# alibaba/nann

Hardware: AMD Instinct MI355X
Metric: retrieval QPS @ recall@200 parity, 1M items/128-d (higher is better)
Workload: dtype f16 rows / f32 L2

## Files before the change

nann_amd/build.py:

```python
import os
import subprocess
import sys

HERE = os.path.dirname(os.path.abspath(__file__))
SRC_DIR = os.path.join(HERE, "csrc")
OUT_DIR = os.path.join(HERE, "_build")
LIB = os.path.join(OUT_DIR, "libnann_hip.so")
UNITS = [("nann_core.o", [("nann_hip.hip", {}), ("nann_comm.hip", {}), ("nann_hnsw_build.hip", {})]),
         ("nann_l2_f16.o", [("nann_l2_inst.hip", {"NANN_L2_DT": "0", "NANN_L2_NAME": "f16"})]),
         ("nann_l2_bf16.o", [("nann_l2_inst.hip", {"NANN_L2_DT": "1", "NANN_L2_NAME": "bf16"})]),
         ("nann_l2_f32.o", [("nann_l2_inst.hip", {"NANN_L2_DT": "2", "NANN_L2_NAME": "f32"})]),
         ("nann_mlp_d64_res.o", [("nann_mlp_inst.hip", {"NANN_MLP_D": "64"}), ("nann_mlp_res_inst.hip", {})]),
         ("nann_mlp_d128.o", [("nann_mlp_inst.hip", {"NANN_MLP_D": "128"})]),
         ("nann_mlp_d256.o", [("nann_mlp_inst.hip", {"NANN_MLP_D": "256"})]),
         ("nann_attn.o", [("nann_attn_inst.hip", {})]),
         ("nann_attn_split.o", [("nann_attn_split_inst.hip", {})]),
         ("nann_eval.o", [("nann_eval_inst.hip", {})]),
         ("nann_eval_lds.o", [("nann_eval_lds_inst.hip", {})]),
         ("nann_eval_win.o", [("nann_eval_win_inst.hip", {})])]
DEPS = ["nann_hip.hip", "nann_mlp_inst.hip", "nann_mlp_res_inst.hip", "nann_mlp5.h", "nann_mlp6.h", "nann_l2_inst.hip", "nann_attn_inst.hip", "nann_attn_split_inst.hip", "nann_attn_split.h", "nann_attn_proj.h", "nann_eval_inst.hip", "nann_eval_lds_inst.hip", "nann_eval_win_inst.hip", "nann_eval.h", "nann_comm.hip", "nann_hnsw_build.hip", "nann_device.h", "nann_mlp.h", "nann_mlp2.h", "nann_mlp3.h",
        "nann_attn.h", "nann_attn_kernels.h", "nann_search.h", os.path.join("host", "nann_graphdef.h"), os.path.join("host", "nann_graphdef_text.h"), os.path.join("host", "nann_blaze_options.h"), os.path.join("host", "nann_npy.h"), os.path.join("host", "nann_projcache.h"),
        os.path.join("..", "..", "include", "nann_hip.h")]
FLAGS = ["-O3", "-std=c++17", "--offload-arch=gfx950", "-fPIC", "-fno-fast-math", "-ffp-contract=off"]


def _hipcc():
    for c in (os.environ.get("HIPCC"), "/opt/rocm/bin/hipcc", "hipcc"):
        if c and (os.path.isabs(c) and os.path.exists(c) or not os.path.isabs(c)):
            return c
    return "hipcc"


def source_hash():
    import hashlib
    h = hashlib.sha256()
    for d in sorted(DEPS):
        with open(os.path.join(SRC_DIR, d), "rb") as f:
            h.update(d.encode() + b"\0" + f.read())
    h.update(" ".join(FLAGS).encode())
    return h.hexdigest()


def is_stale():
    if not os.path.exists(LIB):
        return True
    try:
        with open(LIB + ".srchash") as f:
            return f.read().strip() != source_hash()
    except OSError:
        return True


def build(force=False, verbose=False, variant=None, extra_flags=()):
    if variant is None:
# ... 86 lines not shown
```

nann_amd/csrc/nann_hip.hip:

```cpp
#include "nann_eval.h"
#include "nann_attn.h"
#include "host/nann_graphdef_text.h"
#include "host/nann_blaze_options.h"
#include "host/nann_npy.h"
#include "host/nann_projcache.h"

#include <algorithm>
#include <atomic>
#include <cmath>
#include <cstdio>
#include <cstdlib>
#include <cstring>
#include <fstream>
#include <memory>
#include <mutex>
#include <string>
#include <vector>

#include <sys/stat.h>

using namespace nann;

namespace nann {
thread_local std::string g_err;
int fail(int code, const std::string& msg) {
  g_err = msg;
  return code;
}
}

namespace {

#define HIP_TRY(expr)                                                                    \
  do {                                                                                   \
// ... 578 lines not shown
struct HipProjBackend {
  typedef hipStream_t Stream;
  typedef hipEvent_t Event;
  static bool malloc(void** p, size_t bytes) {
    if (hipMalloc(p, bytes) == hipSuccess) return true;
    (void)hipGetLastError();
    return false;
  }
  static void free(void* p) { (void)hipFree(p); }
  static bool mem_info(size_t* free_b) {
    size_t total = 0;
    if (hipMemGetInfo(free_b, &total) == hipSuccess) return true;
    (void)hipGetLastError();
    return false;
  }
  static bool event_create(Event* e) {
    if (hipEventCreateWithFlags(e, hipEventDisableTiming) == hipSuccess) return true;
    (void)hipGetLastError();
    return false;
  }
  static void event_destroy(Event e) { (void)hipEventDestroy(e); }
  static void event_record(Event e, Stream s) { (void)hipEventRecord(e, s); }
  static bool event_done(Event e) { return hipEventQuery(e) != hipErrorNotReady; }
  static void event_wait(Event e) { (void)hipEventSynchronize(e); }
};
typedef nann::ProjCacheT<HipProjBackend> ProjCache;
typedef nann::ProjTableT<HipProjBackend> ProjTable;
struct SearchOpt {
  int mode;
  int reserve;
  int preproject;
  int mlp_form;
  int small32;
};
static std::atomic<int> g_traversal_mode{-1}, g_slot_reserve{-1}, g_preproject{-1};
static const SearchOpt& env_defaults() {
  static const SearchOpt d = [] {
    SearchOpt o{NANN_TRAVERSAL_AUTO, 0, 1, NANN_MLP_FORM_AUTO, 1};
    if (const char* e = std::getenv("NANN_PREPROJECT")) o.preproject = !(e[0] == '0' && e[1] == 0);
    if (const char* e = std::getenv("NANN_SEARCH_SLOT_RESERVE")) o.reserve = std::max(0, std::atoi(e));
    if (const char* e = std::getenv("NANN_MLP_FORM")) o.mlp_form = std::string(e) == "fused" ? NANN_MLP_FORM_FUSED : std::string(e) == "phased" ? NANN_MLP_FORM_PHASED : NANN_MLP_FORM_AUTO;
    if (const char* e = std::getenv("NANN_PHASE_SMALL32")) o.small32 = !(e[0] == '0');
    return o;
  }();
  return d;
}
static SearchOpt resolve_options(const nann_search_options* u) {
  SearchOpt o = env_defaults();
  const int gm = g_traversal_mode.load(std::memory_order_relaxed), gr = g_slot_reserve.load(std::memory_order_relaxed),
            gp = g_preproject.load(std::memory_order_relaxed);
  if (gm >= 0) o.mode = gm;
  if (gr >= 0) o.reserve = gr;
  if (gp >= 0) o.preproject = gp;
  if (u) {
    const size_t nb = u->struct_bytes > 0 ? (size_t)u->struct_bytes : sizeof(*u);
    auto has = [&](const int32_t* f) { return (size_t)(reinterpret_cast<const char*>(f) - reinterpret_cast<const char*>(u)) + 4 <= nb; };
    if (has(&u->traversal_mode) && u->traversal_mode >= 0) o.mode = u->traversal_mode;
    if (has(&u->slot_reserve) && u->slot_reserve >= 0) o.reserve = u->slot_reserve;
    if (has(&u->preprojection) && u->preprojection >= 0) o.preproject = u->preprojection != 0;
    if (has(&u->mlp_form) && u->mlp_form >= 0) o.mlp_form = u->mlp_form;
  }
  return o;
}
static int check_options(const nann_search_options* u) {
  if (!u) return NANN_OK;
  if (u->struct_bytes < 0 || (u->struct_bytes > 0 && u->struct_bytes < 8)) return fail(NANN_ERR_BAD_ARGUMENT, "nann_search_options: struct_bytes");
  const SearchOpt o = resolve_options(u);
  if (o.mode < NANN_TRAVERSAL_AUTO || o.mode > NANN_TRAVERSAL_LDS_HASH32) return fail(NANN_ERR_BAD_ARGUMENT, "nann_search_options: unknown traversal_mode");
  if (o.mlp_form < NANN_MLP_FORM_AUTO || o.mlp_form > NANN_MLP_FORM_PHASED) return fail(NANN_ERR_BAD_ARGUMENT, "nann_search_options: unknown mlp_form");
  return NANN_OK;
}

struct nann_scorer {
  nann_scorer_desc desc;
  float* dev_weights = nullptr;
  uint4* dev_packed = nullptr;
  float4* dev_packed_x = nullptr;
  MlpParams mlp = {};
  mutable ProjCache proj;
};

struct nann_attn_scorer {
  AttnParams P = {};
  int emb_dtype = 0;
  int precision = NANN_MLP_EXACT_F32;
  float* dev_weights = nullptr;
  uint4* dev_packed = nullptr;
  mutable ProjCache proj;
};

struct nann_index {
  nann_index_desc desc;
  uint64_t uid = 0;
  bool owns = false;
  std::vector<void*> owned;
  int64_t max_deg[2] = {0, 0};
  uint32_t bm_words = 0;
  bool probe_valid = false;
  int probe_ef = 0, probe_queries = 0;
  float probe_new_per_row_mean = 0.0f, probe_new_per_row_q90 = 0.0f, probe_new_per_row_max = 0.0f;
};
static void probe_index(nann_index* ix);

extern "C" {

int nann_abi_version(void) { return NANN_ABI_VERSION; }
const char* nann_last_error(void) { return nann::g_err.c_str(); }

int nann_device_count(void) {
  int n = 0;
  if (hipGetDeviceCount(&n) != hipSuccess) return 0;
  return n;
}

int nann_malloc(void** dev_ptr, int64_t nbytes) {
  if (!dev_ptr || nbytes < 0) return fail(NANN_ERR_BAD_ARGUMENT, "nann_malloc: bad argument");
  HIP_TRY(hipMalloc(dev_ptr, (size_t)std::max<int64_t>(nbytes, 1)));
  return NANN_OK;
}

int nann_free(void* dev_ptr) {
  if (dev_ptr) HIP_TRY(hipFree(dev_ptr));
  return NANN_OK;
}

int nann_memcpy(void* dst, const void* src, int64_t nbytes, int kind, nann_stream_t stream) {
  static const hipMemcpyKind kinds[3] = {hipMemcpyHostToDevice, hipMemcpyDeviceToHost,
                                         hipMemcpyDeviceToDevice};
  if (kind < 0 || kind > 2 || nbytes < 0) return fail(NANN_ERR_BAD_ARGUMENT, "nann_memcpy: bad argument");
  if (nbytes == 0) return NANN_OK;
  HIP_TRY(hipMemcpyAsync(dst, src, (size_t)nbytes, kinds[kind], as_stream(stream)));
  return NANN_OK;
}

int nann_stream_synchronize(nann_stream_t stream) {
// ... 973 lines not shown
    for (int64_t i = 0; i < N; ++i) {
      const int64_t len = rs[(size_t)i + 1] - rs[(size_t)i];
      if (len < 0) { delete ix; return fail(NANN_ERR_INVALID_RAGGED_PARAMS, "row_splits not monotone"); }
      md = std::max(md, len);
    }
    ix->max_deg[l] = md;
  }
  for (int64_t i = 0; i < h.n_enter; ++i) {
    if (ep_host[(size_t)i] < 0 || ep_host[(size_t)i] >= N) { delete ix; return fail(NANN_ERR_INDEX_OUT_OF_RANGE, "enter point out of range"); }
    if (i && ep_host[(size_t)i] <= ep_host[(size_t)i - 1]) { delete ix; return fail(NANN_ERR_BAD_ARGUMENT, "enter points must be ascending and unique"); }
  }
  ix->bm_words = (uint32_t)(((N + 31) / 32 + 3) / 4 * 4);
  if (!h.on_device) {
    auto up = [&](const void* src, size_t bytes, const void** dst) -> int {
      void* d = nullptr;
      HIP_TRY(hipMalloc(&d, std::max<size_t>(bytes, 16)));
      ix->owned.push_back(d);
      if (bytes) HIP_TRY(hipMemcpy(d, src, bytes, hipMemcpyHostToDevice));
      *dst = d;
      return NANN_OK;
    };
    nann_index_desc& dd = ix->desc;
    rc = up(h.item_embs, (size_t)N * h.d * dtype_bytes(h.emb_dtype), &dd.item_embs);
    if (!rc) rc = up(h.item_ids, (size_t)N * 8, reinterpret_cast<const void**>(&dd.item_ids));
    for (int l = 0; l < 2 && !rc; ++l) {
      rc = up(h.nb_values[l], (size_t)h.nb_nnz[l] * 4, reinterpret_cast<const void**>(&dd.nb_values[l]));
      if (!rc) rc = up(h.nb_row_splits[l], (size_t)(N + 1) * 8, reinterpret_cast<const void**>(&dd.nb_row_splits[l]));
    }
    if (!rc) rc = up(h.enter_points, (size_t)h.n_enter * 4, reinterpret_cast<const void**>(&dd.enter_points));
    if (rc) { nann_index_destroy(ix); return rc; }
    ix->owns = true;
    dd.on_device = 1;
  }
  probe_index(ix);
  *out = ix;
  return NANN_OK;
}

void nann_index_destroy(nann_index* ix) {
  if (!ix) return;
  ProjCache::drop_index(ix->uid);
  for (void* p : ix->owned) (void)hipFree(p);
  delete ix;
}

int nann_index_probe_info(const nann_index* ix, float out[5]) {
  if (!ix || !out) return fail(NANN_ERR_BAD_ARGUMENT, "nann_index_probe_info: null argument");
  out[0] = ix->probe_valid ? (float)ix->probe_queries : 0.0f;
  out[1] = (float)ix->probe_ef;
  out[2] = ix->probe_new_per_row_mean;
  out[3] = ix->probe_new_per_row_q90;
  out[4] = ix->probe_new_per_row_max;
  return NANN_OK;
}

int nann_index_info(const nann_index* ix, int64_t out[6]) {
  if (!ix || !out) return fail(NANN_ERR_BAD_ARGUMENT, "nann_index_info: null argument");
  out[0] = ix->desc.n_items; out[1] = ix->desc.d; out[2] = ix->desc.n_enter;
  out[3] = ix->max_deg[0]; out[4] = ix->max_deg[1]; out[5] = ix->bm_words;
  return NANN_OK;
}

constexpr int64_t kPhaseTail = 8192;

static int bit_length(uint64_t v) { int b = 0; while (v) { ++b; v >>= 1; } return b; }

constexpr int kKindAttn = 2;
constexpr int kKindMlpSplit = 3;
constexpr int kKindMlpRes = 4;
static int plan_search(const nann_index* ix, const int32_t t[6], int64_t n_queries, int kind, SearchPlan* p, const SearchOpt& opt,
                       bool mlp_exact_hint = false) {
  for (int i = 0; i < 6; ++i)
    if (t[i] < 0 || t[i] > kMaxK) return fail(NANN_ERR_UNSUPPORTED, "level_topn entries must be in [0, 1024]");
  DeviceInfo di;
  int rc = device_info(&di);
// ... 117 lines not shown
    p->slots = std::max(1, std::min(p->slots, di.cus * per_cu - reserve));
    p->fb_slots = std::max(1, std::min(p->fb_slots, di.cus * bm_per_cu - reserve));
    p->phase_slots = std::max(1, std::min(p->phase_slots, di.cus * p->phase_per_cu - reserve));
    p->phase_score_wgs = std::max(1, di.cus - (reserve + 1) / 2);
  }
  return NANN_OK;
}

int nann_set_search_reserve(int32_t workgroups) {
  if (workgroups < 0) return fail(NANN_ERR_BAD_ARGUMENT, "nann_set_search_reserve: negative");
  g_slot_reserve.store(workgroups, std::memory_order_relaxed);
  return NANN_OK;
}

void nann_search_options_init(nann_search_options* o) {
  if (!o) return;
  o->struct_bytes = (int32_t)sizeof(*o);
  o->traversal_mode = o->slot_reserve = o->preprojection = o->mlp_form = -1;
}

int nann_set_traversal_mode(int32_t mode) {
  if (mode < NANN_TRAVERSAL_AUTO || mode > NANN_TRAVERSAL_LDS_HASH32)
    return fail(NANN_ERR_BAD_ARGUMENT, "nann_set_traversal_mode: unknown mode");
  g_traversal_mode.store(mode, std::memory_order_relaxed);
  return NANN_OK;
}

int nann_search_workspace_bytes(const nann_index* ix, const int32_t level_topn[6], int64_t n_queries,
                                int64_t* nbytes) {
  if (!ix || !level_topn || !nbytes) return fail(NANN_ERR_BAD_ARGUMENT, "nann_search_workspace_bytes: null argument");
  SearchPlan p;
  const int rc = plan_search(ix, level_topn, n_queries, -1, &p, resolve_options(nullptr));
  if (rc) return rc;
  *nbytes = (int64_t)(256 + p.slot_bytes * (unsigned long long)std::max(p.slots, p.fb_slots) + kPhaseTail);
  return NANN_OK;
}

}


template <typename Build>
static int projection_for(ProjCache& c, const nann_index* ix, int width, hipStream_t st, Build build, bool pin, bool enabled,
                          std::shared_ptr<ProjTable>* out) {
  const size_t bytes = (size_t)ix->desc.n_items * (size_t)width * 4;
  return c.acquire(ix->uid, bytes, enabled, pin, [&](float* t) -> int {
    const int rc = build(t);
    if (rc) return rc;
    const hipError_t e = hipStreamSynchronize(st);
    if (e != hipSuccess) return fail(NANN_ERR_HIP, std::string("pre-projection: ") + hipGetErrorString(e));
    return NANN_OK;
  }, out);
}

static void projection_used(ProjCache& c, const std::shared_ptr<ProjTable>& tab, hipStream_t st) { c.used(tab, st); }

static int projection_release(ProjCache& c, const nann_index* ix) {
  if (c.release(ix->uid)) return NANN_OK;
  return fail(NANN_ERR_BAD_ARGUMENT, "release: no pre-projected table of this index");
}

static int mlp_projection(const nann_scorer* sc, const nann_index* ix, hipStream_t st, bool pin, bool enabled, std::shared_ptr<ProjTable>* out) {
  return projection_for(sc->proj, ix, kMlpProjWidth, st, [&](float* t) {
    return launch_mlp_preproject(ix->desc.emb_dtype, ix->desc.item_embs, (long long)ix->desc.n_items, ix->desc.d, sc->mlp.w1, t, st);
  }, pin, enabled, out);
}

static int attn_projection(const nann_attn_scorer* sc, const nann_index* ix, hipStream_t st, bool pin, bool enabled, std::shared_ptr<ProjTable>* out) {
// ... 69 lines not shown
  }
  const int64_t need_slots = p.phased ? std::max<int64_t>(std::min<int64_t>(n_queries, kPhaseChunk), p.fb_slots) : std::max(p.slots, p.fb_slots);
  if (!workspace || workspace_bytes < (int64_t)(256 + p.slot_bytes * (unsigned long long)need_slots + (p.phased ? kPhaseTail : 0)))
    return fail(NANN_ERR_CAPACITY, "workspace smaller than nann_search_workspace_bytes()");
  SearchArgs a;
  a.emb = ix->desc.item_embs;
  a.item_ids = ix->desc.item_ids;
  for (int l = 0; l < 2; ++l) { a.nbv[l] = ix->desc.nb_values[l]; a.nbrs[l] = ix->desc.nb_row_splits[l]; }
  a.enter = ix->desc.enter_points;
  a.n_enter = (int)ix->desc.n_enter;
  a.n_items = (uint32_t)ix->desc.n_items;
  a.d = ix->desc.d;
  a.q = q;
  a.n_queries = (int)n_queries;
  for (int i = 0; i < 6; ++i) a.t[i] = level_topn[i];
  a.tq = tq;
  a.ws = static_cast<unsigned char*>(workspace);
  a.slot_bytes = p.slot_bytes;
  a.bm_words = ix->bm_words;
  a.max_cand = p.max_cand; a.max_raw = p.max_raw; a.pool_cap = p.pool_cap;
  a.out_ids = out_item_ids; a.out_scores = out_scores; a.out_index = out_index;
  a.status = status; a.counters = counters;
  a.phase_ticks = reinterpret_cast<long long*>(phase_ticks);
  a.id_bits = p.id_bits;
  a.redo = 0;
  a.phase = 0;
  a.proj = tab ? tab->table : nullptr;
  a.mlp = MlpParams{};
  a.attn = AttnParams{};
  a.kt = kt; a.upad = upad;
  HIP_TRY(hipMemsetAsync(workspace, 0, 256, st));
  const int dt = ix->desc.emb_dtype;
  const bool hashed = p.vis == VIS_LDS_HASH || p.vis == VIS_LDS_HASH32;
  auto both = [&](auto&& launch_on) -> int {
    int r2 = launch_on(p.vis, p.nt, p.slots, p.lds_bytes);
    if (!r2 && hashed) {
      a.redo = 1;
      r2 = launch_on(p.fb_vis, kNT, p.fb_slots, p.fb_lds_bytes);
    }
    if (cache) projection_used(*cache, tab, st);
    return r2;
  };
  if (attn) {
    a.attn = attn->P;
    if (tab) {
      auto launch = attn->precision == NANN_MLP_SPLIT_F16 ? launch_search_attn_proj : launch_search_attn_xproj;
      const bool resident = attn->precision == NANN_MLP_SPLIT_F16;
      return both([&](int vis, int, int slots, size_t lds) {
        if (resident && vis == VIS_LDS_HASH && !a.redo) return launch_search_attn_res(slots, lds, a, st);
        return launch(vis, slots, lds, a, st);
      });
    }
    auto launch = attn->precision == NANN_MLP_SPLIT_F16 ? launch_search_attn_split : launch_search_attn;
    return both([&](int vis, int, int slots, size_t lds) { return launch(ix->desc.d, dt, vis, slots, lds, a, st); });
  }
  a.mlp = scorer->mlp;
  a.phase = 0;
  const int exact = scorer->desc.kind == NANN_SCORER_MLP && scorer->desc.precision == NANN_MLP_EXACT_F32;
  if (mlp_res && p.phased) {
    DeviceInfo di;
    rc = device_info(&di);
    if (rc) return rc;
    const int k5 = level_topn[5];
    for (int64_t c0 = 0; c0 < n_queries && !rc; c0 += kPhaseChunk) {
      SearchArgs c = a;
      c.n_queries = (int)std::min<int64_t>(kPhaseChunk, n_queries - c0);
      c.q = q + (size_t)c0 * a.d;
      if (tq) c.tq = tq + (size_t)c0 * 6;
      c.out_ids = out_item_ids + (size_t)c0 * k5;
      if (out_scores) c.out_scores = out_scores + (size_t)c0 * k5;
// ... 10 lines not shown
          rc = launch_mlp_phase_score(exact, c, ph, p.phase_score_wgs, st);
        }
      }
      if (!rc) {
        c.redo = 1;
        c.phase = 0;
        rc = launch_search_mlp_res(exact, p.fb_vis, p.fb_slots, p.fb_lds_bytes, c, st);
      }
    }
    if (cache) projection_used(*cache, tab, st);
    return rc;
  }
  if (mlp_res)
    return both([&](int vis, int, int slots, size_t lds) {
      return launch_search_mlp_res(exact, vis, slots, lds, a, st);
    });
  return both([&](int vis, int nt, int slots, size_t lds) {
    return launch_search_any(ix->desc.d / 8, dt, kind, mlp_split, vis, nt, slots, lds, a, st);
  });
}

__global__ void k_probe_queries(const void* emb, int dt, int d, long long n_items, int nq, float* q) {
  const int j = blockIdx.x;
  const long long row = (long long)j * (n_items / nq);
  for (int k = threadIdx.x; k < d; k += blockDim.x) {
    float v;
    if (dt == NANN_F32) v = static_cast<const float*>(emb)[row * d + k];
    else {
      const uint32_t h = static_cast<const uint16_t*>(emb)[row * d + k];
      v = dt == NANN_F16 ? half_bits_to_float(h) : bf16_bits_to_float(h);
    }
    q[(size_t)j * d + k] = v;
  }
}

static void probe_index(nann_index* ix) {
  ix->probe_valid = false;
  static const bool enabled = [] { const char* e = std::getenv("NANN_INDEX_PROBE"); return !(e && e[0] == '0'); }();
  if (!enabled) return;
  const std::string saved_error = nann::g_err;
  struct RestoreError { const std::string& s; ~RestoreError() { nann::g_err = s; } } restore{saved_error};
  const int d = ix->desc.d;
  const int64_t E = ix->desc.n_enter, N = ix->desc.n_items;
  if (E < 8 || N < 4096) return;
  const int nq = 64, e = (int)std::min<int64_t>(64, E);
  const int32_t t[6] = {e, e, e, e, e, std::min(e, 10)};
  nann_scorer_desc sd{};
  sd.kind = NANN_SCORER_L2; sd.d = d; sd.emb_dtype = ix->desc.emb_dtype;
  nann_scorer* sc = nullptr;
  if (nann_scorer_create(&sd, &sc) != NANN_OK) return;
  nann_search_options o;
  nann_search_options_init(&o);
  o.traversal_mode = NANN_TRAVERSAL_HBM_BITMAP;
  o.slot_reserve = 0;
  int64_t ws_bytes = 0;
  const size_t n_ctr = (size_t)nq * 3 * NANN_NUM_ROUNDS;
  unsigned char* buf = nullptr;
  std::vector<int32_t> h_ctr(n_ctr), h_st((size_t)nq);
  bool ok = nann_search_workspace_bytes(ix, t, nq, &ws_bytes) == NANN_OK;
  const size_t off_q = ((size_t)ws_bytes + 255) & ~(size_t)255, off_ids = off_q + (size_t)nq * d * 4,
               off_st = off_ids + (size_t)nq * t[5] * 8, off_ctr = off_st + (size_t)nq * 4, total = off_ctr + n_ctr * 4;
  ok = ok && hipMalloc(reinterpret_cast<void**>(&buf), total) == hipSuccess;
  if (ok) {
    hipStream_t st = nullptr;
    hipLaunchKernelGGL(k_probe_queries, dim3(nq), dim3(128), 0, st, ix->desc.item_embs, ix->desc.emb_dtype, d, (long long)N, nq,
                       reinterpret_cast<float*>(buf + off_q));
// ... 99 lines not shown
  if (resident_bytes) {
    *resident_bytes = 0;
    ProjCache* c = at ? &at->proj : s ? &s->proj : nullptr;
    if (c) *resident_bytes = (int64_t)c->resident();
  }
  return NANN_OK;
}

int nann_scorer_prepare(const nann_scorer* scorer, const nann_index* ix, nann_stream_t stream) {
  if (!scorer || !ix) return fail(NANN_ERR_BAD_ARGUMENT, "nann_scorer_prepare: null argument");
  return prepare_impl(scorer, nullptr, ix, as_stream(stream));
}
int nann_scorer_release(const nann_scorer* scorer, const nann_index* ix) {
  if (!scorer || !ix) return fail(NANN_ERR_BAD_ARGUMENT, "nann_scorer_release: null argument");
  if (table_width(scorer, nullptr) == 0) return NANN_OK;
  return projection_release(scorer->proj, ix);
}
int nann_scorer_table_bytes(const nann_scorer* scorer, const nann_index* ix, int64_t* table_bytes, int64_t* resident_bytes) {
  if (!scorer) return fail(NANN_ERR_BAD_ARGUMENT, "nann_scorer_table_bytes: null scorer");
  return table_bytes_impl(scorer, nullptr, ix, table_bytes, resident_bytes);
}

static size_t model_query_bytes(const nann_model* m, int64_t n_queries) {
  const size_t per = m->kind == NANN_MODEL_ATTENTION ? (size_t)(256 * 64 + 64 * 64) * 4 : (size_t)m->d * 4;
  return ((size_t)n_queries * per + 255) & ~(size_t)255;
}

int nann_search_model_workspace_bytes(const nann_index* ix, const nann_model* m, const int32_t level_topn[6],
                                      int64_t n_queries, int64_t* nbytes) {
  if (!ix || !m || !level_topn || !nbytes) return fail(NANN_ERR_BAD_ARGUMENT, "nann_search_model_workspace_bytes: null argument");
  SearchPlan p;
  const int rc = plan_search(ix, level_topn, n_queries, m->kind == NANN_MODEL_ATTENTION ? kKindAttn : -1, &p, resolve_options(nullptr));
  if (rc) return rc;
  *nbytes = (int64_t)(256 + p.slot_bytes * (unsigned long long)std::max(p.slots, p.fb_slots) + kPhaseTail + 256 +
                      model_query_bytes(m, n_queries));
  return NANN_OK;
}

static int search_model_impl(const nann_index* ix, const nann_model* m, const void* comm_seq_f16, int64_t n_queries,
                             const int32_t level_topn[6], const int32_t* tq, void* workspace, int64_t workspace_bytes,
                             int64_t* out_item_ids, float* out_scores, int32_t* out_index, int32_t* status,
                             int32_t* counters, const nann_search_options* options, nann_search_plan* plan, nann_stream_t stream) {
  if (!ix || !m || !comm_seq_f16 || !level_topn || !out_item_ids || !status || !workspace)
    return fail(NANN_ERR_BAD_ARGUMENT, "nann_search_model: null argument");
  if (n_queries <= 0) return NANN_OK;
  if (m->d != ix->desc.d || m->emb_dtype != ix->desc.emb_dtype)
    return fail(NANN_ERR_BAD_ARGUMENT, "model and index disagree on d / dtype");
  int64_t need = 0;
  int rc = nann_search_model_workspace_bytes(ix, m, level_topn, n_queries, &need);
  if (rc) return rc;
  if (workspace_bytes < need) return fail(NANN_ERR_CAPACITY, "workspace smaller than nann_search_model_workspace_bytes()");
  const size_t qb = model_query_bytes(m, n_queries);
  const int64_t search_bytes = need - (int64_t)qb - 256;
  unsigned char* qbuf = static_cast<unsigned char*>(workspace) + ((search_bytes + 255) & ~255ll);
  hipStream_t st = as_stream(stream);
  if (m->kind == NANN_MODEL_ATTENTION) {
    float* kt = reinterpret_cast<float*>(qbuf);
    float* upad = kt + (size_t)n_queries * 256 * 64;
    rc = nann_attn_prepare(m->attn, comm_seq_f16, n_queries, kt, upad, stream);
    if (rc) return rc;
    return search_impl(ix, nullptr, m->attn, nullptr, kt, upad, n_queries, level_topn, tq, workspace, search_bytes,
                       out_item_ids, out_scores, out_index, status, counters, nullptr, options, plan, st);
  }
  float* q = reinterpret_cast<float*>(qbuf);
  rc = nann_user_seq_mean(comm_seq_f16, n_queries, m->seq_len, m->d, q, stream);
  if (rc) return rc;
  return search_impl(ix, m->scorer, nullptr, q, nullptr, nullptr, n_queries, level_topn, tq, workspace, search_bytes,
                     out_item_ids, out_scores, out_index, status, counters, nullptr, options, plan, st);
// ... 256 lines not shown
```

nann_amd/csrc/nann_search.h:

```cpp
#pragma once
#ifndef NANN_REPEAT_SCORE
#define NANN_REPEAT_SCORE 0
#endif
#ifndef NANN_REPEAT_TOPK
#define NANN_REPEAT_TOPK 0
#endif
#include <type_traits>
#include "../../include/nann_hip.h"
#include "nann_device.h"
#include "nann_mlp.h"
#include "nann_mlp2.h"
#include "nann_mlp3.h"
#include "nann_mlp5.h"
#include "nann_mlp6.h"
#include "nann_attn_kernels.h"
#include "nann_attn_split.h"
#include "nann_attn_proj.h"

#include <string>

namespace nann {

struct OpResult {
  long long n_out;
  long long n_out_splits;
  long long bad_i;
  int code;
  int err;
};


int fail(int code, const std::string& msg);

#define NANN_HIP_TRY(expr)                                                                 \
  do {                                                                                     \
    hipError_t _e = (expr);                                                                \
    if (_e != hipSuccess)                                                                  \
      return ::nann::fail(NANN_ERR_HIP, std::string(#expr) + ": " + hipGetErrorString(_e)); \
  } while (0)

template <int D, int DT, bool SPLIT>
__global__ __launch_bounds__(kMlpNT) void k_score_mlp(MlpParams P, const void* table, long long n_table_rows,
// ... 50 lines not shown
}

struct SearchArgs {
  const void* emb;
  const int64_t* item_ids;
  const int32_t* nbv[2];
  const int64_t* nbrs[2];
  const int32_t* enter;
  int n_enter;
  uint32_t n_items;
  int d;
  const float* q;
  int n_queries;
  int t[6];
  const int32_t* tq;
  unsigned char* ws;
  unsigned long long slot_bytes;
  uint32_t bm_words;
  int max_cand, max_raw, pool_cap;
  int64_t* out_ids;
  float* out_scores;
  int32_t* out_index;
  int32_t* status;
  int32_t* counters;
  long long* phase_ticks;
  MlpParams mlp;
  const float* proj;
  AttnParams attn;
  const float* kt;
  const float* upad;
  int id_bits;
  int redo;
  int phase;
};

static_assert(PH_COUNT == NANN_NUM_PHASES, "phase list out of sync with include/nann_hip.h");

struct SlotView {
  int32_t* cand_ids;
  float* cand_scores;
  int32_t* raw;
  int32_t* beam_ids;
  float* beam_scores;
  int32_t* pool_ids;
  float* pool_scores;
  uint32_t* gbitmap;
  PhaseState* phase;
};

__host__ __device__ inline unsigned long long slot_layout(int max_cand, int max_raw, int pool_cap,
                                                          uint32_t gbm_words, unsigned long long off[9]) {
  unsigned long long o = 0;
  auto put = [&](int i, unsigned long long bytes) { off[i] = o; o += (bytes + 255ull) & ~255ull; };
  put(0, 4ull * max_cand);
  put(1, 4ull * max_cand);
  put(2, 4ull * max_raw);
  put(3, 4ull * kMaxK);
  put(4, 4ull * kMaxK);
  put(5, 4ull * pool_cap);
  put(6, 4ull * pool_cap);
  put(8, sizeof(PhaseState));
  put(7, 4ull * gbm_words);
  return o;
}

constexpr int kScorerMlpSplit = 2;
// ... 394 lines not shown
  int32_t* s_ctr = misc + 2;
  long long* s_ticks = reinterpret_cast<long long*>(misc + 20);

  unsigned long long off[9];
  slot_layout(a.max_cand, a.max_raw, a.pool_cap, VIS == VIS_HBM_BITMAP ? a.bm_words : 0u, off);
  constexpr bool PHASED = SC == kScorerMlpPhase;
  SlotView sv;
  auto bind_slot = [&](unsigned long long index) {
  unsigned char* slot = a.ws + 256 + index * a.slot_bytes;
  sv.cand_ids = reinterpret_cast<int32_t*>(slot + off[0]);
  sv.cand_scores = reinterpret_cast<float*>(slot + off[1]);
  sv.raw = reinterpret_cast<int32_t*>(slot + off[2]);
  sv.beam_ids = reinterpret_cast<int32_t*>(slot + off[3]);
  sv.beam_scores = reinterpret_cast<float*>(slot + off[4]);
  sv.pool_ids = reinterpret_cast<int32_t*>(slot + off[5]);
  sv.pool_scores = reinterpret_cast<float*>(slot + off[6]);
  sv.gbitmap = reinterpret_cast<uint32_t*>(slot + off[7]);
  sv.phase = reinterpret_cast<PhaseState*>(slot + off[8]);
  };
  bind_slot(blockIdx.x);
  uint32_t* bm = VIS == VIS_HBM_BITMAP ? sv.gbitmap : bm_lds;
  const int k5 = a.t[5];
  WsHeader* hdr = reinterpret_cast<WsHeader*>(a.ws);
  if (a.redo) {
    if (__hip_atomic_load(&hdr->n_redo, __ATOMIC_RELAXED, __HIP_MEMORY_SCOPE_AGENT) == 0u) return;
  }
  unsigned int* queue = a.redo ? &hdr->redo_queue : PHASED ? &hdr->pqueue[a.phase] : &hdr->queue;
  if constexpr (is_mlp_res(SC)) {
    const uint4* w2 = SC == kScorerMlpXRes ? reinterpret_cast<const uint4*>(a.mlp.p2x) : a.mlp.p2;
    constexpr int keep_from = mlp_res_reload_bytes(HASH) / 16;
    for (int i = keep_from + (int)threadIdx.x; i < kMlpResW2Vec; i += NT) reinterpret_cast<uint4*>(smem)[i] = w2[i];
  }

  for (;;) {
    __syncthreads();
    if (threadIdx.x == 0) {
      int qn = (int)atomicAdd(queue, 1u);
      if (a.redo)
        while (qn < a.n_queries && a.status[qn] != NANN_ERR_CAPACITY) qn = (int)atomicAdd(queue, 1u);
      misc[0] = qn;
    }
    if (threadIdx.x < 3 * NANN_NUM_ROUNDS) s_ctr[threadIdx.x] = 0;
    if (threadIdx.x < NANN_NUM_PHASES) s_ticks[threadIdx.x] = 0;
    __syncthreads();
    const int qi = misc[0];
    if (qi >= a.n_queries) break;
    if constexpr (PHASED) bind_slot((unsigned long long)qi);
    const int st = search_one<LPR, DT, VIS, SC, NT>(a, qi, sv, bm, scratch, qv, s_ctr, s_ticks);
    __syncthreads();
    if constexpr (PHASED) {
      if (st == kPhaseSkip) continue;
      if (threadIdx.x == 0) sv.phase->status = st;
      if (a.phase_ticks && threadIdx.x < NANN_NUM_PHASES) {
        long long* dst = &a.phase_ticks[(size_t)qi * NANN_NUM_PHASES + threadIdx.x];
        s_ticks[threadIdx.x] += a.phase ? *dst : 0;
        if (st == kPhasePending) *dst = s_ticks[threadIdx.x];
      }
      if (st == kPhasePending) continue;
    }
    const int k_done = st ? 0 : (a.tq ? a.tq[(size_t)qi * 6 + 5] : k5);
    if (k_done < k5) {
      for (int i = k_done + (int)threadIdx.x; i < k5; i += NT) {
        a.out_ids[(size_t)qi * k5 + i] = 0;
        if (a.out_scores) a.out_scores[(size_t)qi * k5 + i] = 0.0f;
        if (a.out_index) a.out_index[(size_t)qi * k5 + i] = 0;
      }
    }
    if (threadIdx.x == 0) {
      a.status[qi] = st;
      if (HASH && st == NANN_ERR_CAPACITY) atomicAdd(&hdr->n_redo, 1u);
    }
    if (a.counters && threadIdx.x < 3 * NANN_NUM_ROUNDS)
// ... 70 lines not shown
```

Measured before the change: 2.549 million.

## Cluster queries by nearest pivot and route clusters to per-XCD work queues

At index build, a farthest-point set of pivots is chosen from entry points. At search time, each query is assigned to its nearest pivot, and a counting-sort kernel builds a permutation. Search blocks pull queries from per-XCC segments of that permutation, so queries that likely visit similar graph regions run on the same XCD and share its L2 cache. This adds two small kernels per search and a fixed segment schedule that may balance load worse than the single global queue.

```diff
diff --git a/nann_amd/build.py b/nann_amd/build.py
--- a/nann_amd/build.py
+++ b/nann_amd/build.py
@@ -19,7 +19,7 @@
          ("nann_eval_lds.o", [("nann_eval_lds_inst.hip", {})]),
          ("nann_eval_win.o", [("nann_eval_win_inst.hip", {})])]
 DEPS = ["nann_hip.hip", "nann_mlp_inst.hip", "nann_mlp_res_inst.hip", "nann_mlp5.h", "nann_mlp6.h", "nann_l2_inst.hip", "nann_attn_inst.hip", "nann_attn_split_inst.hip", "nann_attn_split.h", "nann_attn_proj.h", "nann_eval_inst.hip", "nann_eval_lds_inst.hip", "nann_eval_win_inst.hip", "nann_eval.h", "nann_comm.hip", "nann_hnsw_build.hip", "nann_device.h", "nann_mlp.h", "nann_mlp2.h", "nann_mlp3.h",
-        "nann_attn.h", "nann_attn_kernels.h", "nann_search.h", os.path.join("host", "nann_graphdef.h"), os.path.join("host", "nann_graphdef_text.h"), os.path.join("host", "nann_blaze_options.h"), os.path.join("host", "nann_npy.h"), os.path.join("host", "nann_projcache.h"),
+        "nann_attn.h", "nann_attn_kernels.h", "nann_search.h", "nann_order.h", "nann_order_kernels.h", os.path.join("host", "nann_graphdef.h"), os.path.join("host", "nann_graphdef_text.h"), os.path.join("host", "nann_blaze_options.h"), os.path.join("host", "nann_npy.h"), os.path.join("host", "nann_projcache.h"),
         os.path.join("..", "..", "include", "nann_hip.h")]
 FLAGS = ["-O3", "-std=c++17", "--offload-arch=gfx950", "-fPIC", "-fno-fast-math", "-ffp-contract=off"]
 
diff --git a/nann_amd/csrc/nann_hip.hip b/nann_amd/csrc/nann_hip.hip
--- a/nann_amd/csrc/nann_hip.hip
+++ b/nann_amd/csrc/nann_hip.hip
@@ -1,5 +1,6 @@
 #include "nann_eval.h"
 #include "nann_attn.h"
+#include "nann_order_kernels.h"
 #include "host/nann_graphdef_text.h"
 #include "host/nann_blaze_options.h"
 #include "host/nann_npy.h"
@@ -644,15 +645,17 @@
   int preproject;
   int mlp_form;
   int small32;
+  int order;
 };
 static std::atomic<int> g_traversal_mode{-1}, g_slot_reserve{-1}, g_preproject{-1};
 static const SearchOpt& env_defaults() {
   static const SearchOpt d = [] {
-    SearchOpt o{NANN_TRAVERSAL_AUTO, 0, 1, NANN_MLP_FORM_AUTO, 1};
+    SearchOpt o{NANN_TRAVERSAL_AUTO, 0, 1, NANN_MLP_FORM_AUTO, 1, 1};
     if (const char* e = std::getenv("NANN_PREPROJECT")) o.preproject = !(e[0] == '0' && e[1] == 0);
     if (const char* e = std::getenv("NANN_SEARCH_SLOT_RESERVE")) o.reserve = std::max(0, std::atoi(e));
     if (const char* e = std::getenv("NANN_MLP_FORM")) o.mlp_form = std::string(e) == "fused" ? NANN_MLP_FORM_FUSED : std::string(e) == "phased" ? NANN_MLP_FORM_PHASED : NANN_MLP_FORM_AUTO;
     if (const char* e = std::getenv("NANN_PHASE_SMALL32")) o.small32 = !(e[0] == '0');
+    if (const char* e = std::getenv("NANN_QUERY_ORDER")) o.order = !(e[0] == '0');
     return o;
   }();
   return d;
@@ -711,8 +714,13 @@
   bool probe_valid = false;
   int probe_ef = 0, probe_queries = 0;
   float probe_new_per_row_mean = 0.0f, probe_new_per_row_q90 = 0.0f, probe_new_per_row_max = 0.0f;
+  float* pivots = nullptr;
+  int n_pivots = 0;
 };
 static void probe_index(nann_index* ix);
+static void choose_pivots(nann_index* ix, const std::vector<int32_t>& enter);
+static int launch_order(const nann_index* ix, const float* q, int n, int32_t* key, int32_t* perm, unsigned int* heads,
+                        hipStream_t st);
 
 extern "C" {
 
@@ -1752,6 +1760,7 @@
     ix->owns = true;
     dd.on_device = 1;
   }
+  choose_pivots(ix, ep_host);
   probe_index(ix);
   *out = ix;
   return NANN_OK;
@@ -1761,6 +1770,7 @@
   if (!ix) return;
   ProjCache::drop_index(ix->uid);
   for (void* p : ix->owned) (void)hipFree(p);
+  if (ix->pivots) (void)hipFree(ix->pivots);
   delete ix;
 }
 
@@ -1944,7 +1954,8 @@
   SearchPlan p;
   const int rc = plan_search(ix, level_topn, n_queries, -1, &p, resolve_options(nullptr));
   if (rc) return rc;
-  *nbytes = (int64_t)(256 + p.slot_bytes * (unsigned long long)std::max(p.slots, p.fb_slots) + kPhaseTail);
+  *nbytes = (int64_t)(256 + p.slot_bytes * (unsigned long long)std::max(p.slots, p.fb_slots) + kPhaseTail +
+                      order_ws_bytes(n_queries));
   return NANN_OK;
 }
 
@@ -2080,10 +2091,25 @@
   HIP_TRY(hipMemsetAsync(workspace, 0, 256, st));
   const int dt = ix->desc.emb_dtype;
   const bool hashed = p.vis == VIS_LDS_HASH || p.vis == VIS_LDS_HASH32;
+  const unsigned long long slots_end = 256 + p.slot_bytes * (unsigned long long)std::max(p.slots, p.fb_slots) + kPhaseTail;
+  const unsigned long long order_off = ((unsigned long long)workspace_bytes - order_ws_bytes(n_queries)) & ~255ull;
+  if (opt.order && hashed && !attn && kind == NANN_SCORER_L2 && ix->n_pivots >= 2 && n_queries > p.slots &&
+      (unsigned long long)workspace_bytes >= ((slots_end + 255) & ~255ull) + order_ws_bytes(n_queries)) {
+    unsigned char* ow = static_cast<unsigned char*>(workspace) + order_off;
+    unsigned int* heads = reinterpret_cast<unsigned int*>(ow);
+    int32_t* perm = reinterpret_cast<int32_t*>(ow + kOrderSegs * kOrderHeadStride * 4);
+    int32_t* key = perm + n_queries;
+    rc = launch_order(ix, q, (int)n_queries, key, perm, heads, st);
+    if (rc) return rc;
+    a.perm = perm;
+    a.xheads = heads;
+  }
   auto both = [&](auto&& launch_on) -> int {
     int r2 = launch_on(p.vis, p.nt, p.slots, p.lds_bytes);
     if (!r2 && hashed) {
       a.redo = 1;
+      a.perm = nullptr;
+      a.xheads = nullptr;
       r2 = launch_on(p.fb_vis, kNT, p.fb_slots, p.fb_lds_bytes);
     }
     if (cache) projection_used(*cache, tab, st);
@@ -2160,6 +2186,78 @@
     }
     q[(size_t)j * d + k] = v;
   }
+}
+
+__global__ void k_order_gather(const void* emb, int dt, int d, const int32_t* rows, int m, float* out) {
+  for (int k = threadIdx.x; k < d; k += blockDim.x) out[(size_t)blockIdx.x * d + k] = order_row_elem(emb, dt, (size_t)rows[blockIdx.x] * d + k);
+}
+
+static int launch_order(const nann_index* ix, const float* q, int n, int32_t* key, int32_t* perm, unsigned int* heads,
+                        hipStream_t st) {
+  const int d = ix->desc.d, P = ix->n_pivots;
+  const size_t lds = ((size_t)d * P + kOrderMaxPivots + (size_t)kOrderKeyQueries * d) * 4;
+  if (lds > 48 * 1024)
+    HIP_TRY(hipFuncSetAttribute(reinterpret_cast<const void*>(k_order_key), hipFuncAttributeMaxDynamicSharedMemorySize, (int)lds));
+  hipLaunchKernelGGL(k_order_key, dim3((unsigned)((n + kOrderKeyQueries - 1) / kOrderKeyQueries)), dim3(256), lds, st,
+                     ix->pivots, d, P, q, n, key);
+  HIP_TRY(hipGetLastError());
+  hipLaunchKernelGGL(k_order_perm, dim3(1), dim3(kOrderSortThreads), 0, st, key, n, P, perm, heads);
+  HIP_TRY(hipGetLastError());
+  return NANN_OK;
+}
+
+static void choose_pivots(nann_index* ix, const std::vector<int32_t>& enter) {
+  const int d = ix->desc.d;
+  const int P = order_pivots((int64_t)enter.size(), d);
+  if (P < 2) return;
+  constexpr size_t kMaxCand = 1024;
+  const size_t E = enter.size(), m = std::min(E, kMaxCand);
+  std::vector<int32_t> cand(m);
+  for (size_t i = 0; i < m; ++i) cand[i] = enter[i * E / m];
+  int32_t* rows = nullptr;
+  float* buf = nullptr;
+  std::vector<float> x(m * (size_t)d);
+  bool ok = hipMalloc(&rows, m * 4) == hipSuccess && hipMalloc(&buf, m * (size_t)d * 4) == hipSuccess &&
+            hipMemcpy(rows, cand.data(), m * 4, hipMemcpyHostToDevice) == hipSuccess;
+  if (ok) {
+    hipLaunchKernelGGL(k_order_gather, dim3((unsigned)m), dim3(128), 0, nullptr, ix->desc.item_embs, ix->desc.emb_dtype, d, rows, (int)m, buf);
+    ok = hipGetLastError() == hipSuccess && hipMemcpy(x.data(), buf, x.size() * 4, hipMemcpyDeviceToHost) == hipSuccess;
+  }
+  if (buf) (void)hipFree(buf);
+  if (rows) (void)hipFree(rows);
+  if (!ok) return;
+  std::vector<size_t> piv;
+  std::vector<double> dist(m, INFINITY);
+  size_t cur = 0;
+  for (int p = 0; p < P; ++p) {
+    piv.push_back(cur);
+    size_t far = cur;
+    for (size_t i = 0; i < m; ++i) {
+      double s = 0.0;
+      for (int k = 0; k < d; ++k) { const double t = (double)x[i * d + k] - (double)x[cur * d + k]; s += t * t; }
+      dist[i] = std::min(dist[i], s);
+      if (dist[i] > dist[far]) far = i;
+    }
+    if (dist[far] <= 0.0) break;
+    cur = far;
+  }
+  if (piv.size() < 2) return;
+  const size_t np = piv.size();
+  std::vector<float> t((size_t)d * np + kOrderMaxPivots, 0.0f);
+  for (size_t p = 0; p < np; ++p) {
+    float s = 0.0f;
+    for (int k = 0; k < d; ++k) {
+      const float v = x[piv[p] * d + k];
+      t[(size_t)k * np + p] = v;
+      s += v * v;
+    }
+    t[(size_t)d * np + p] = s;
+  }
+  float* dev = nullptr;
+  if (hipMalloc(&dev, t.size() * 4) != hipSuccess) return;
+  if (hipMemcpy(dev, t.data(), t.size() * 4, hipMemcpyHostToDevice) != hipSuccess) { (void)hipFree(dev); return; }
+  ix->pivots = dev;
+  ix->n_pivots = (int)piv.size();
 }
 
 static void probe_index(nann_index* ix) {
@@ -2325,8 +2423,8 @@
   SearchPlan p;
   const int rc = plan_search(ix, level_topn, n_queries, m->kind == NANN_MODEL_ATTENTION ? kKindAttn : -1, &p, resolve_options(nullptr));
   if (rc) return rc;
-  *nbytes = (int64_t)(256 + p.slot_bytes * (unsigned long long)std::max(p.slots, p.fb_slots) + kPhaseTail + 256 +
-                      model_query_bytes(m, n_queries));
+  *nbytes = (int64_t)(256 + p.slot_bytes * (unsigned long long)std::max(p.slots, p.fb_slots) + kPhaseTail +
+                      order_ws_bytes(n_queries) + 256 + model_query_bytes(m, n_queries));
   return NANN_OK;
 }
 
diff --git a/nann_amd/csrc/nann_order.h b/nann_amd/csrc/nann_order.h
--- /dev/null
+++ b/nann_amd/csrc/nann_order.h
@@ -0,0 +1,38 @@
+#pragma once
+#include <hip/hip_runtime.h>
+#include <hip/hip_fp16.h>
+#include <stdint.h>
+#include <algorithm>
+#include <cmath>
+#include "../../include/nann_hip.h"
+
+namespace nann {
+
+constexpr int kOrderSegs = 8;
+constexpr int kOrderHeadStride = 32;
+constexpr int kOrderMaxPivots = 128;
+constexpr int kOrderPivotLds = 64 * 1024;
+constexpr int kOrderKeyQueries = 16;
+constexpr int kOrderSortThreads = 1024;
+
+__host__ __device__ inline int order_seg_begin(int n, int s) { return (int)((long long)n * s / kOrderSegs); }
+
+inline int order_pivots(int64_t n_enter, int d) {
+  return (int)std::min<int64_t>(n_enter, std::min(kOrderMaxPivots, kOrderPivotLds / (4 * d)));
+}
+
+inline unsigned long long order_ws_bytes(int64_t n) {
+  return ((unsigned long long)kOrderSegs * kOrderHeadStride * 4 + (unsigned long long)n * 8 + 255) / 256 * 256;
+}
+
+__device__ inline unsigned int xcc_id() {
+#if defined(__HIP_DEVICE_COMPILE__)
+  unsigned int x;
+  asm volatile("s_getreg_b32 %0, hwreg(HW_REG_XCC_ID, 0, 4)" : "=s"(x));
+  return x;
+#else
+  return 0;
+#endif
+}
+
+}
diff --git a/nann_amd/csrc/nann_order_kernels.h b/nann_amd/csrc/nann_order_kernels.h
--- /dev/null
+++ b/nann_amd/csrc/nann_order_kernels.h
@@ -0,0 +1,97 @@
+#pragma once
+#include "nann_order.h"
+
+namespace nann {
+
+__device__ inline float order_row_elem(const void* emb, int dt, size_t i) {
+  if (dt == NANN_F32) return reinterpret_cast<const float*>(emb)[i];
+  const uint16_t h = reinterpret_cast<const uint16_t*>(emb)[i];
+  if (dt == NANN_F16) return __half2float(__ushort_as_half(h));
+  return __uint_as_float((uint32_t)h << 16);
+}
+
+__global__ __launch_bounds__(256) void k_order_key(const float* pivT, int d, int P, const float* q, int n, int32_t* key) {
+  extern __shared__ float4 order_lds4[];
+  float* piv = reinterpret_cast<float*>(order_lds4);
+  float* qs = piv + (size_t)d * P + kOrderMaxPivots;
+  const int q0 = blockIdx.x * kOrderKeyQueries, nq = min(kOrderKeyQueries, n - q0);
+  const int pv4 = (d * P + kOrderMaxPivots) / 4, qv4 = nq * d / 4;
+  for (int i = threadIdx.x; i < pv4; i += 256) order_lds4[i] = reinterpret_cast<const float4*>(pivT)[i];
+  for (int i = threadIdx.x; i < qv4; i += 256)
+    reinterpret_cast<float4*>(qs)[i] = reinterpret_cast<const float4*>(q + (size_t)q0 * d)[i];
+  __syncthreads();
+  const int lane = threadIdx.x & 63, wave = threadIdx.x >> 6;
+  const int pa = lane, pb = lane + 64;
+  float acc[4][2] = {};
+  const float* qw = qs + (size_t)wave * 4 * d;
+  for (int k = 0; k < d; ++k) {
+    const float va = piv[k * P + min(pa, P - 1)], vb = piv[k * P + min(pb, P - 1)];
+#pragma unroll
+    for (int j = 0; j < 4; ++j) {
+      const float x = qw[j * d + k];
+      acc[j][0] = fmaf(x, va, acc[j][0]);
+      acc[j][1] = fmaf(x, vb, acc[j][1]);
+    }
+  }
+  const float* pn = piv + (size_t)d * P;
+#pragma unroll
+  for (int j = 0; j < 4; ++j) {
+    const int qi = wave * 4 + j;
+    float best = pa < P ? fmaf(-2.0f, acc[j][0], pn[min(pa, P - 1)]) : INFINITY;
+    int arg = pa < P ? pa : 0x7fffffff;
+    if (pb < P) {
+      const float s = fmaf(-2.0f, acc[j][1], pn[pb]);
+      if (s < best) { best = s; arg = pb; }
+    }
+    for (int m = 32; m >= 1; m >>= 1) {
+      const float ob = __shfl_xor(best, m);
+      const int oa = __shfl_xor(arg, m);
+      if (ob < best || (ob == best && oa < arg)) { best = ob; arg = oa; }
+    }
+    if (lane == 0 && qi < nq) key[q0 + qi] = arg < P ? arg : 0;
+  }
+}
+
+__global__ __launch_bounds__(kOrderSortThreads) void k_order_perm(const int32_t* key, int n, int P, int32_t* perm,
+                                                                 unsigned int* heads) {
+  constexpr int W = kOrderSortThreads / 64;
+  __shared__ int base[kOrderMaxPivots];
+  __shared__ int wofs[W][kOrderMaxPivots];
+  const int tid = threadIdx.x, lane = tid & 63, w = tid >> 6;
+  if (tid < kOrderSegs * kOrderHeadStride) heads[tid] = 0u;
+  for (int p = tid; p < P; p += blockDim.x) base[p] = 0;
+  __syncthreads();
+  for (int i = tid; i < n; i += blockDim.x) atomicAdd(&base[key[i]], 1);
+  __syncthreads();
+  int pre = 0;
+  if (tid < P)
+    for (int p = 0; p < tid; ++p) pre += base[p];
+  __syncthreads();
+  if (tid < P) base[tid] = pre;
+  __syncthreads();
+  for (int t0 = 0; t0 < n; t0 += kOrderSortThreads) {
+    for (int i = tid; i < W * kOrderMaxPivots; i += blockDim.x) (&wofs[0][0])[i] = 0;
+    __syncthreads();
+    const int i = t0 + tid;
+    const int k = i < n ? key[i] : -1;
+    int rank = 0;
+    bool last = true;
+#pragma unroll
+    for (int j = 0; j < 64; ++j) {
+      const int kj = __builtin_amdgcn_readlane(k, j);
+      if (kj == k) { if (j < lane) ++rank; else if (j > lane) last = false; }
+    }
+    if (k >= 0 && last) wofs[w][k] = rank + 1;
+    __syncthreads();
+    for (int p = tid; p < P; p += blockDim.x) {
+      int run = base[p];
+      for (int v = 0; v < W; ++v) { const int c = wofs[v][p]; wofs[v][p] = run; run += c; }
+      base[p] = run;
+    }
+    __syncthreads();
+    if (k >= 0) perm[wofs[w][k] + rank] = i;
+    __syncthreads();
+  }
+}
+
+}
diff --git a/nann_amd/csrc/nann_search.h b/nann_amd/csrc/nann_search.h
--- a/nann_amd/csrc/nann_search.h
+++ b/nann_amd/csrc/nann_search.h
@@ -8,6 +8,7 @@
 #include <type_traits>
 #include "../../include/nann_hip.h"
 #include "nann_device.h"
+#include "nann_order.h"
 #include "nann_mlp.h"
 #include "nann_mlp2.h"
 #include "nann_mlp3.h"
@@ -124,6 +125,8 @@
   int id_bits;
   int redo;
   int phase;
+  const int32_t* perm = nullptr;
+  unsigned int* xheads = nullptr;
 };
 
 static_assert(PH_COUNT == NANN_NUM_PHASES, "phase list out of sync with include/nann_hip.h");
@@ -584,12 +587,25 @@
     for (int i = keep_from + (int)threadIdx.x; i < kMlpResW2Vec; i += NT) reinterpret_cast<uint4*>(smem)[i] = w2[i];
   }
 
+  int seg = 0;
+  unsigned int xcd = 0;
+  if (a.perm && threadIdx.x == 0) xcd = xcc_id() % kOrderSegs;
   for (;;) {
     __syncthreads();
     if (threadIdx.x == 0) {
-      int qn = (int)atomicAdd(queue, 1u);
-      if (a.redo)
-        while (qn < a.n_queries && a.status[qn] != NANN_ERR_CAPACITY) qn = (int)atomicAdd(queue, 1u);
+      int qn = a.n_queries;
+      if (a.perm) {
+        for (; seg < kOrderSegs; ++seg) {
+          const unsigned int s = (xcd + (unsigned int)seg) % kOrderSegs;
+          const int lo = order_seg_begin(a.n_queries, (int)s), n = order_seg_begin(a.n_queries, (int)s + 1) - lo;
+          const int pos = (int)atomicAdd(&a.xheads[s * kOrderHeadStride], 1u);
+          if (pos < n) { qn = a.perm[lo + pos]; break; }
+        }
+      } else {
+        qn = (int)atomicAdd(queue, 1u);
+        if (a.redo)
+          while (qn < a.n_queries && a.status[qn] != NANN_ERR_CAPACITY) qn = (int)atomicAdd(queue, 1u);
+      }
       misc[0] = qn;
     }
     if (threadIdx.x < 3 * NANN_NUM_ROUNDS) s_ctr[threadIdx.x] = 0;
```

After: 2.797 million, median of 6. 9.7% higher.
